# duckietown/gym-duckietown

Measured on NVIDIA H100. Metric: env-steps/sec (obs+reward+done) at N envs, 1/2/4/8 H100 vs CPU ref, higher is better.
Workload: dtype f64 logic / f32 raster / u8 obs

## Files before the change

### gym-duckietown_b200/csrc/dts_render.cu

```cuda
#include <algorithm>
#include <cstddef>
#include <cstdlib>
#include <type_traits>
#include <vector>

#include "dts_camera.cuh"
#include "dts_kernels.h"

namespace dts {

struct FishTab {
  const int32_t* src_xy;
  const short4* cbox;
  const short4* fbox;
  const int32_t* cell_start;
  const uint16_t* cell_bins;
  const int32_t* home_start;
  const int4* home_ent;
  int ext_x, ext_y;
};

struct PilTab {
  int W, H, ow, oh;
  int tx, ty;
  int band, cap;
  int pitch, ow3p;
  size_t smem;
  int32_t* tab;
};

namespace {

#ifndef DTS_STATS
#define DTS_STATS 0
#endif
#if DTS_STATS
#define DTS_COUNT(slot, n) do { if (lane == 0) atomicAdd(err + (slot), (n)); } while (0)
#else
#define DTS_COUNT(slot, n) do { } while (0)
#endif
constexpr int kThreads = 256;
constexpr int kRasterMinCtas = 3;
constexpr int kSoloMinCtas = 3;
constexpr int kFlatMinCtas = 4;
constexpr int kGeoWarps = 1;
constexpr int kGeoMinCtas = 32;
constexpr int kWarps = kThreads / 32;
constexpr int kBinW = 8, kBinH = 4;
constexpr int kCFX = 4, kCFY = 2;
constexpr int kCoarseW = kBinW * kCFX, kCoarseH = kBinH * kCFY;
constexpr int kStage = 32;
constexpr float kGuard = 4.0f;
constexpr int kSub = 64;
constexpr int kTessTris = 98;
__host__ __device__ constexpr int tile_draw_ids(bool tess) { return tess ? kTessTris : 2; }
__host__ __device__ constexpr int agent_item(int n_tiles, int n_objects) { return 1 + n_tiles + n_objects; }
__host__ __device__ constexpr int sample_x(int s) { return s == 0 ? 24 : (s == 1 ? 56 : (s == 2 ? 8 : 40)); }
__host__ __device__ constexpr int sample_y(int s) { return s == 0 ? 8 : (s == 1 ? 24 : (s == 2 ? 40 : 56)); }

struct Vtx { float cx, cy, cz, cw, r, g, b, u, v; };

struct __align__(16) PrimRec {
  int32_t X0, Y0, X1, Y1;
  int32_t X2, Y2, X3, Y3;
  float z0, zx, zy;
  int32_t id;
  float q0, qx, qy, u0;
  float ux, uy, v0, vx;
  float vy;
  int32_t ltq;
  uint32_t tex;
  float r0;
  float rx, ry, g0, gx;
  float gy, b0, bx, by;
};
static_assert(sizeof(PrimRec) == 128, "PrimRec must be 128 bytes");
static_assert(offsetof(PrimRec, q0) == 48 && offsetof(PrimRec, vy) == 80 && offsetof(PrimRec, rx) == 96, "PrimRec word groups");

struct __align__(16) BinRec {
  int32_t E0[4], A[4], B[4];
  float z0, zx, zy;
  int32_t id;
  int32_t x0, y0;
  uint32_t prim_flags;
  int32_t kind;
};
static_assert(sizeof(BinRec) == 80, "BinRec layout");
constexpr int kKindQuad = 1;
constexpr int kKindGround = 2;
constexpr int kKindTiny = 4;
constexpr int kKindFlat = 8;
constexpr unsigned kNoPrim = 0xffffu;

struct Xform { float MV[12], N[9]; };

struct __align__(16) FrameCtx {
  double V[12];
  float P00, P11, P22, P23;
  int32_t n_prims, n_lat, overflow, pad;
};

struct __align__(16) GeoWarp {
  int32_t unlit, pad_[3];
  RenderEp ep;
  double V[12];
  float P00, P11, P22, P23;
  Xform x;
  Vtx corners[4];
  Vtx poly[2][12];
};
using Shared = GeoWarp;

__device__ __forceinline__ void model_view(const double* V, double tx, double ty, double tz, double sc, double c,
                                           double s, Xform& x, int lane) {
  __syncwarp();
  if (lane < 12) {
    const int r = lane >> 2, k = lane & 3;
    if (k < 3) {
      const double R0 = k == 0 ? c : (k == 1 ? 0.0 : s), R1 = k == 1 ? 1.0 : 0.0, R2 = k == 0 ? -s : (k == 1 ? 0.0 : c);
      const double a = V[4 * r + 0] * R0 + V[4 * r + 1] * R1 + V[4 * r + 2] * R2;
      x.MV[4 * r + k] = (float)(a * sc);
      x.N[3 * r + k] = (float)(sc == 1.0 ? a : a / sc);
    } else {
      x.MV[4 * r + 3] = (float)(V[4 * r + 0] * tx + V[4 * r + 1] * ty + V[4 * r + 2] * tz + V[4 * r + 3]);
    }
  }
  __syncwarp();
}


__device__ __forceinline__ Vtx shade_vertex(const Xform& x, const Shared& sh, float px, float py, float pz, float nx,
                                            float ny, float nz, float cr, float cg, float cb, float u, float v) {
  float e[3], ne[3];
#pragma unroll
  for (int r = 0; r < 3; r++) {
    float t = x.MV[4 * r] * px;
    t = t + x.MV[4 * r + 1] * py;
    t = t + x.MV[4 * r + 2] * pz;
    e[r] = t + x.MV[4 * r + 3];
    float q = x.N[3 * r] * nx;
    q = q + x.N[3 * r + 1] * ny;
    ne[r] = q + x.N[3 * r + 2] * nz;
  }
  const float* lp = sh.ep.light_eye;
  float lx, ly, lz;
  if (lp[3] == 0.0f) { lx = lp[0]; ly = lp[1]; lz = lp[2]; }
  else { lx = lp[0] - e[0]; ly = lp[1] - e[1]; lz = lp[2] - e[2]; }
  float len = lx * lx;
  len = len + ly * ly;
  len = len + lz * lz;
  len = sqrtf(len);
  float ndl = 0.0f;
  if (len > 0.0f) {
    lx = lx / len; ly = ly / len; lz = lz / len;
    ndl = ne[0] * lx;
    ndl = ndl + ne[1] * ly;
    ndl = ndl + ne[2] * lz;
    if (!(ndl > 0.0f)) ndl = 0.0f;
  }
  Vtx o;
  const float col[3] = {cr, cg, cb};
  float lit[3];
#pragma unroll
  for (int k = 0; k < 3; k++) {
    float s = 0.3f + sh.ep.ambient[k];
    s = s + ndl * sh.ep.diffuse[k];
    const float c = sh.unlit ? col[k] : col[k] * s;
    lit[k] = c < 0.0f ? 0.0f : (c > 1.0f ? 1.0f : c);
  }
  o.r = lit[0]; o.g = lit[1]; o.b = lit[2];
  o.u = u; o.v = v;
  o.cx = sh.P00 * e[0];
  o.cy = sh.P11 * e[1];
  o.cz = sh.P22 * e[2] + sh.P23;
  o.cw = -e[2];
  return o;
}

__device__ __forceinline__ float plane_dist(const Vtx& a, int pl) {
  switch (pl) {
    case 0: return a.cz + a.cw;
    case 1: return a.cw - a.cz;
    case 2: return a.cx + kGuard * a.cw;
    case 3: return kGuard * a.cw - a.cx;
    case 4: return a.cy + kGuard * a.cw;
    default: return kGuard * a.cw - a.cy;
  }
}

__device__ __forceinline__ int classify(const Vtx& a, const Vtx& b, const Vtx& c) {
  const Vtx* v[3] = {&a, &b, &c};
  int out[6] = {0, 0, 0, 0, 0, 0}, need = 0;
#pragma unroll
  for (int k = 0; k < 3; k++) {
    const float x = v[k]->cx, y = v[k]->cy, z = v[k]->cz, w = v[k]->cw;
    out[0] += !(z + w >= 0.0f); out[1] += !(w - z >= 0.0f);
    out[2] += x < -w; out[3] += x > w; out[4] += y < -w; out[5] += y > w;
    need |= !(x + kGuard * w >= 0.0f) | !(kGuard * w - x >= 0.0f) | !(y + kGuard * w >= 0.0f) |
            !(kGuard * w - y >= 0.0f);
  }
  need |= out[0] | out[1];
#pragma unroll
  for (int p = 0; p < 6; p++) if (out[p] == 3) return 2;
  return need ? 1 : 0;
}

struct EmitCtx {
  const DTexture* textures;
  GeoWarp* gw;
  FrameCtx* ctx;
  PrimRec* prims;
  int max_prims, W, H;
};

__device__ __noinline__ bool setup_and_emit(const EmitCtx& ec, const Vtx& a, const Vtx& b, const Vtx& c, int id,
                                            int tex, int lat, const Vtx* d = nullptr) {
  const Vtx* vs[3] = {&a, &b, &c};
  int X[3], Y[3];
  float zw[3], q[3];
  const float Wf = (float)ec.W, Hf = (float)ec.H;
#pragma unroll
  for (int k = 0; k < 3; k++) {
    const float iw = 1.0f / vs[k]->cw;
    const float nx = vs[k]->cx * iw, ny = vs[k]->cy * iw, nz = vs[k]->cz * iw;
    const float sx = (nx * 0.5f + 0.5f) * Wf;
    const float sy = (0.5f - ny * 0.5f) * Hf;
    X[k] = (int)rintf(sx * 64.0f);
    Y[k] = (int)rintf(sy * 64.0f);
    zw[k] = nz * 0.5f + 0.5f;
    q[k] = iw;
  }
// ... 25 lines not shown
    const int ex[3] = {x1 - x0, x2 - x1, x0 - x2}, ey[3] = {y1 - y0, y2 - y1, y0 - y2};
    const int ax[3] = {0, x1 - x0, x2 - x0}, ay[3] = {0, y1 - y0, y2 - y0};
    int e00[3];
#pragma unroll
    for (int k = 0; k < 3; k++) {
      const int bias = (ey[k] > 0 || (ey[k] == 0 && ex[k] < 0)) ? 0 : 1;
      e00[k] = ex[k] * (py0 * kSub - y0 - ay[k]) - ey[k] * (px0 * kSub - x0 - ax[k]) - bias;
    }
    bool any = false;
    for (int py = 0; py <= py1 - py0; py++)
      for (int px = 0; px <= px1 - px0; px++) {
#pragma unroll
        for (int s = 0; s < 4; s++) {
          const int sx = px * kSub + sample_x(s), sy = py * kSub + sample_y(s);
          const int e0 = e00[0] + ex[0] * sy - ey[0] * sx, e1 = e00[1] + ex[1] * sy - ey[1] * sx, e2 = e00[2] + ex[2] * sy - ey[2] * sx;
          any |= (e0 | e1 | e2) >= 0;
        }
      }
    if (!any) return true;
  }
  PrimRec r;
  r.X0 = x0; r.Y0 = y0; r.X1 = x1; r.Y1 = y1; r.X2 = x2; r.Y2 = y2; r.X3 = x0; r.Y3 = y0;
  const float dx1 = (float)(x1 - x0) * 0.015625f, dy1 = (float)(y1 - y0) * 0.015625f;
  const float dx2 = (float)(x2 - x0) * 0.015625f, dy2 = (float)(y2 - y0) * 0.015625f;
  const float areaf = dx1 * dy2 - dx2 * dy1;
  const float ia = 1.0f / areaf;
  const Vtx* p0 = vs[0]; const Vtx* p1 = vs[i1]; const Vtx* p2 = vs[i2];
  const float q0 = q[0], q1 = q[i1], q2 = q[i2];
  const float v0[7] = {zw[0], q0, p0->u * q0, p0->v * q0, p0->r * q0, p0->g * q0, p0->b * q0};
  const float v1[7] = {zw[i1], q1, p1->u * q1, p1->v * q1, p1->r * q1, p1->g * q1, p1->b * q1};
  const float v2[7] = {zw[i2], q2, p2->u * q2, p2->v * q2, p2->r * q2, p2->g * q2, p2->b * q2};
  float f0[7], fx[7], fy[7];
#pragma unroll
  for (int at = 0; at < 7; at++) {
    const float d1 = v1[at] - v0[at], d2 = v2[at] - v0[at];
    f0[at] = v0[at];
    fx[at] = (d1 * dy2 - d2 * dy1) * ia;
    fy[at] = (d2 * dx1 - d1 * dx2) * ia;
  }
  r.z0 = f0[0]; r.zx = fx[0]; r.zy = fy[0];
  r.q0 = f0[1]; r.qx = fx[1]; r.qy = fy[1];
  r.u0 = f0[2]; r.ux = fx[2]; r.uy = fy[2];
  r.v0 = f0[3]; r.vx = fx[3]; r.vy = fy[3];
  r.r0 = f0[4]; r.rx = fx[4]; r.ry = fy[4];
  r.g0 = f0[5]; r.gx = fx[5]; r.gy = fy[5];
  r.b0 = f0[6]; r.bx = fx[6]; r.by = fy[6];
  r.id = id;
  r.ltq = (lat + 1) | ((tex + 1) << 16);
  r.tex = tex >= 0 ? ec.textures[tex].info : 0u;
  if (d) {
    r.ltq |= 1 << 24;
    r.X1 = qx[1]; r.Y1 = qy[1]; r.X2 = qx[2]; r.Y2 = qy[2]; r.X3 = qx[3]; r.Y3 = qy[3];
  }
  const int slot = atomicAdd(&ec.ctx->n_prims, 1);
  if (slot >= ec.max_prims) { ec.ctx->overflow = 1; return true; }
  const int4* src = reinterpret_cast<const int4*>(&r);
  int4* dst = reinterpret_cast<int4*>(ec.prims + slot);
#pragma unroll
  for (int k = 0; k < 8; k++) dst[k] = src[k];
  return true;
}

__device__ __forceinline__ Vtx clip_lerp(const Vtx& in, const Vtx& out, float din, float dout) {
  const float t = din / (din - dout);
  Vtx o;
  const float* a = reinterpret_cast<const float*>(&in);
  const float* b = reinterpret_cast<const float*>(&out);
  float* c = reinterpret_cast<float*>(&o);
#pragma unroll
  for (int k = 0; k < 9; k++) { const float d = b[k] - a[k]; c[k] = a[k] + t * d; }
  return o;
}

__device__ __forceinline__ void clip_and_emit_warp(const EmitCtx& ec, const Vtx& a, const Vtx& b, const Vtx& c, int id,
                                                   int tex, int lat, int lane) {
  for (int p2 = 0; p2 < 6; p2++) {
    const int cnt = !(plane_dist(a, p2) >= 0.0f) + !(plane_dist(b, p2) >= 0.0f) + !(plane_dist(c, p2) >= 0.0f);
    if (cnt == 3) return;
  }
  GeoWarp& g = *ec.gw;
  __syncwarp();
  if (lane == 0) { g.poly[0][0] = a; g.poly[0][1] = b; g.poly[0][2] = c; }
  __syncwarp();
  int n = 3, cur = 0;
  for (int pl = 0; pl < 6; pl++) {
    const Vtx* P = g.poly[cur];
    const float dk = lane < n ? plane_dist(P[lane], pl) : 0.0f;
    const bool in1 = dk >= 0.0f;
    const unsigned valid = (1u << n) - 1u;
    const unsigned out_mask = __ballot_sync(0xffffffffu, lane < n && !in1);
    if (!out_mask) continue;
    const int k2 = (lane + 1 == n) ? 0 : lane + 1;
    const float dn = __shfl_sync(0xffffffffu, dk, k2 & 31);
    const bool in2 = dn >= 0.0f;
    const bool cross = lane < n && (in1 != in2);
    const unsigned keep_mask = __ballot_sync(0xffffffffu, lane < n && in1) & valid;
    const unsigned cross_mask = __ballot_sync(0xffffffffu, cross) & valid;
    const unsigned below = (1u << lane) - 1u;
    int pos = __popc(keep_mask & below) + __popc(cross_mask & below);
    Vtx* T = g.poly[cur ^ 1];
    if (lane < n) {
      if (in1) T[pos++] = P[lane];
      if (in1 && !in2) T[pos] = clip_lerp(P[lane], P[k2], dk, dn);
      else if (!in1 && in2) T[pos] = clip_lerp(P[k2], P[lane], dn, dk);
    }
    n = __popc(keep_mask) + __popc(cross_mask);
    cur ^= 1;
// ... 446 lines not shown
  out |= (P11 * cy_ + cz_) * hy > rad * 1.01f;
  out |= (-P11 * cy_ + cz_) * hy > rad * 1.01f;
  return out;
}
__device__ __forceinline__ void eye_point(const double* V, double wx, double wy, double wz, float& ex, float& ey, float& ez) {
  ex = (float)(V[0] * wx + V[1] * wy + V[2] * wz + V[3]);
  ey = (float)(V[4] * wx + V[5] * wy + V[6] * wz + V[7]);
  ez = (float)(V[8] * wx + V[9] * wy + V[10] * wz + V[11]);
}

struct ItemPose { int dyn_kind; float opx, opz, orot; bool agent_item; };
__device__ __forceinline__ bool item_visible(const DState& S, const DMap& m, const RenderCfg& rc, const FrameCtx& ctx, int env,
                                             int item, ItemPose& ip) {
  const int n_tiles = m.grid_w * m.grid_h;
  ip.dyn_kind = 0; ip.opx = 0.f; ip.opz = 0.f; ip.orot = 0.f;
  ip.agent_item = item == agent_item(n_tiles, m.n_objects);
  if (item > agent_item(n_tiles, m.n_objects)) return false;
  if (ip.agent_item && (!(rc.mode & DTS_RENDER_TOP_DOWN) || m.agent.tri_count == 0)) return false;
  if (item >= 1 && item <= n_tiles) {
    const int t = item - 1, ti = t / m.grid_h, tj = t - ti * m.grid_h;
    if (m.tile_kind[tj * m.grid_w + ti] < 0) return false;
    const double ts = m.tile_size;
    float ex, ey, ez;
    eye_point(ctx.V, (ti + 0.5) * ts, 0.0, (tj + 0.5) * ts, ex, ey, ez);
    if (sphere_outside(ctx.P00, ctx.P11, ex, ey, ez, (float)(ts * 0.7071067811865476) * 1.001f + 1e-4f)) return false;
  } else if (item > n_tiles) {
    const int o = item - 1 - n_tiles;
    if (!ip.agent_item && (S.rep[env].hidden[o >> 5] >> (o & 31) & 1u)) return false;
    const DObject& ob = ip.agent_item ? m.agent : m.objects[o];
    ip.opx = ob.pos[0]; ip.opz = ob.pos[2]; ip.orot = ob.y_rot_deg;
    if (ip.agent_item) {
      ip.opx = (float)S.pos_x[env]; ip.opz = (float)S.pos_z[env];
      ip.orot = (float)(S.angle[env] * 180.0 / 3.141592653589793);
    }
    if (ob.dyn_slot >= 0) {
      ip.dyn_kind = m.dyn[ob.dyn_slot].kind;
      if (ip.dyn_kind != DTS_DYN_TRAFFICLIGHT) {
        const size_t nd = m.n_dyn, ne = rc.n_envs;
        ip.opx = (float)m.dyn_state[((size_t)DTS_DYN_PX * nd + ob.dyn_slot) * ne + env];
        ip.opz = (float)m.dyn_state[((size_t)DTS_DYN_PZ * nd + ob.dyn_slot) * ne + env];
        ip.orot = (float)m.dyn_state[((size_t)DTS_DYN_YROT * nd + ob.dyn_slot) * ne + env];
      }
    }
    double sn, cs;
    sincos((double)ip.orot * kDeg2Rad, &sn, &cs);
    const double sc = (double)ob.scale, ccx = ob.centre[0], ccy = ob.centre[1], ccz = ob.centre[2];
    float ex, ey, ez;
    eye_point(ctx.V, (double)ip.opx + sc * (cs * ccx + sn * ccz), (double)ob.pos[1] + sc * ccy, (double)ip.opz + sc * (-sn * ccx + cs * ccz), ex, ey, ez);
    if (sphere_outside(ctx.P00, ctx.P11, ex, ey, ez, ob.bound_rad * ob.scale * 1.002f + 2e-4f)) return false;
  }
  return true;
}

__global__ void __launch_bounds__(256) k_cull(const DState S, const DMap* __restrict__ maps, RenderCfg rc, FrameMem fm, int items_max) {
  const size_t g = blockIdx.x * (size_t)blockDim.x + threadIdx.x;
  const int item = (int)(g / rc.n_envs), slot = (int)(g - (size_t)item * rc.n_envs);
  bool vis = false;
  int env = 0;
  if (item < items_max && slot < n_listed(rc.env_list, rc.env_count, rc.n_envs)) {
    env = listed_env(rc.env_list, slot);
    ItemPose ip;
    vis = item_visible(S, maps[S.map_id[env]], rc, fm.ctx[env], env, item, ip);
  }
  const unsigned m = __ballot_sync(0xffffffffu, vis);
  if (!m) return;
  const int lane = threadIdx.x & 31;
  int base = 0;
  if (lane == __ffs(m) - 1) base = atomicAdd(fm.work + kWorkGeoList, __popc(m));
  base = __shfl_sync(0xffffffffu, base, __ffs(m) - 1);
  if (vis) fm.geo_list[base + __popc(m & ((1u << lane) - 1u))] = make_uint2((unsigned)env, (unsigned)item);
}

template <bool kTess>
__device__ __forceinline__ void geometry_item(const DState& S, const DMap* __restrict__ maps, const RenderCfg& rc, const FrameMem& fm,
                                              int max_prims, int max_lat, int32_t* __restrict__ err, int env, int item, int lane,
                                              GeoWarp& sh) {
  const DMap& m = maps[S.map_id[env]];
  const int n_tiles = m.grid_w * m.grid_h;
  const bool seg = (rc.mode & DTS_RENDER_SEGMENT) != 0;
  const int W = rc.width, H = rc.height;
  FrameCtx& ctx = fm.ctx[env];
  ItemPose ip;
  if (!item_visible(S, m, rc, ctx, env, item, ip)) return;
  const bool agent_item = ip.agent_item;
  const int dyn_kind = ip.dyn_kind;
  const float opx = ip.opx, opz = ip.opz, orot = ip.orot;
  __syncwarp();
  for (int k = lane; k < (int)(sizeof(RenderEp) / 4); k += 32)
    reinterpret_cast<uint32_t*>(&sh.ep)[k] = reinterpret_cast<const uint32_t*>(&S.rep[env])[k];
  if (lane < 12) sh.V[lane] = ctx.V[lane];
  if (lane == 12) { sh.P00 = ctx.P00; sh.P11 = ctx.P11; sh.P22 = ctx.P22; sh.P23 = ctx.P23; sh.unlit = seg ? 1 : 0; }
  __syncwarp();
  EmitCtx ec{m.textures, &sh, &ctx, fm.prims + (size_t)env * max_prims, max_prims, W, H};
  float4* lat_tab = fm.lat + (size_t)env * max_lat * 64;
  const int tris_per_tile = tile_draw_ids(kTess);
  Xform& x = sh.x;
  if (item == 0) {
    model_view(sh.V, 0.0, 0.0, 0.0, 1.0, 1.0, 0.0, x, lane);
    const float gy = (float)(-0.8 * 0.01);
    const float P[4][3] = {{-50.f, gy, 50.f}, {-50.f, gy, -50.f}, {50.f, gy, -50.f}, {50.f, gy, 50.f}};
    const float magenta[3] = {255.f, 0.f, 255.f};
    const float* g = seg ? magenta : sh.ep.ground;
    const int pl_ = lane & 3;
    const Vtx mine = shade_vertex(x, sh, P[pl_][0], P[pl_][1], P[pl_][2], 0.f, 1.f, 0.f, g[0], g[1], g[2], 0.f, 0.f);
    if (lane < 4) sh.corners[lane] = mine;
    __syncwarp();
    process_triangle_uniform(ec, sh.corners[0], sh.corners[1], sh.corners[2], 0, -1, -1, lane);
    process_triangle_uniform(ec, sh.corners[0], sh.corners[2], sh.corners[3], 1, -1, -1, lane);
  } else if (item <= n_tiles) {
    const int t = item - 1, ti = t / m.grid_h, tj = t - ti * m.grid_h;
    const int idx = tj * m.grid_w + ti;
    const int quarter = (m.tile_angle[idx] + 2) & 3;
    const double cs = quarter == 0 ? 1.0 : (quarter == 2 ? -1.0 : 0.0), sn = quarter == 1 ? 1.0 : (quarter == 3 ? -1.0 : 0.0);
    const double ts = m.tile_size;
    model_view(sh.V, (double)(float)((ti + 0.5) * ts), 0.0, (double)(float)((tj + 0.5) * ts), 1.0, cs, sn, x, lane);
    int tex = m.tile_tex[idx];
    if (seg && tex >= 0) tex = m.tex_segment[tex];
    const int base_id = 2 + tris_per_tile * t;
    if (!kTess) {
      const int ca = (lane == 1 || lane == 2) ? 7 : 0, cb = (lane >= 2) ? 7 : 0;
      const float lx = (float)(-ts / 2 + ((double)ca / 7.0) * ts), lz = (float)(-ts / 2 + ((double)cb / 7.0) * ts);
      const Vtx v = shade_vertex(x, sh, lx, 0.0f, lz, 0.f, 1.f, 0.f, 1.f, 1.f, 1.f, (float)((double)ca / 7.0),
                                 (float)(1.0 - (double)cb / 7.0));
      const unsigned four = 0xFu;
      bool culled4 = false;
      culled4 |= (__ballot_sync(0xffffffffu, !(v.cz + v.cw >= 0.0f)) & four) == four;
      culled4 |= (__ballot_sync(0xffffffffu, !(v.cw - v.cz >= 0.0f)) & four) == four;
      culled4 |= (__ballot_sync(0xffffffffu, v.cx < -v.cw) & four) == four;
      culled4 |= (__ballot_sync(0xffffffffu, v.cx > v.cw) & four) == four;
      culled4 |= (__ballot_sync(0xffffffffu, v.cy < -v.cw) & four) == four;
      culled4 |= (__ballot_sync(0xffffffffu, v.cy > v.cw) & four) == four;
      if (culled4) return;
    }
    Vtx lv[2];
    int outside[6] = {0, 0, 0, 0, 0, 0};
#pragma unroll
    for (int h = 0; h < 2; h++) {
      const int vi = lane + 32 * h, a = vi >> 3, b = vi & 7;
      const float lx = (float)(-ts / 2 + ((double)a / 7.0) * ts), lz = (float)(-ts / 2 + ((double)b / 7.0) * ts);
      lv[h] = shade_vertex(x, sh, lx, 0.0f, lz, 0.f, 1.f, 0.f, 1.f, 1.f, 1.f, (float)((double)a / 7.0),
                           (float)(1.0 - (double)b / 7.0));
      const Vtx& v = lv[h];
      outside[0] += !(v.cz + v.cw >= 0.0f); outside[1] += !(v.cw - v.cz >= 0.0f);
      outside[2] += v.cx < -v.cw; outside[3] += v.cx > v.cw; outside[4] += v.cy < -v.cw; outside[5] += v.cy > v.cw;
    }
    if (kTess) {
      bool culled = false;
#pragma unroll
      for (int p = 0; p < 6; p++) culled |= __all_sync(0xffffffffu, outside[p] == 2);
      if (culled) return;
    }
    if (!kTess) {
      int slot = 0;
      if (lane == 0) slot = atomicAdd(&ctx.n_lat, 1);
      slot = __shfl_sync(0xffffffffu, slot, 0);
      if (slot >= max_lat) { if (lane == 0) ctx.overflow = 1; return; }
#pragma unroll
      for (int h = 0; h < 2; h++) {
        const int vi = lane + 32 * h;
        lat_tab[slot * 64 + vi] = make_float4(lv[h].r, lv[h].g, lv[h].b, 0.0f);
        int corner = -1;
        if (vi == 0) corner = 0; else if (vi == 56) corner = 1; else if (vi == 63) corner = 2; else if (vi == 7) corner = 3;
        if (corner >= 0) { Vtx c = lv[h]; c.r = 0.f; c.g = 0.f; c.b = 0.f; sh.corners[corner] = c; }
      }
      __syncwarp();
      bool as_quad = false;
      if (classify(sh.corners[0], sh.corners[1], sh.corners[2]) == 0 && classify(sh.corners[0], sh.corners[2], sh.corners[3]) == 0) {
        if (lane == 0) as_quad = setup_and_emit(ec, sh.corners[0], sh.corners[1], sh.corners[2], base_id, tex, slot, &sh.corners[3]);
        as_quad = __shfl_sync(0xffffffffu, (int)as_quad, 0) != 0;
      }
      if (!as_quad) {
        process_triangle_uniform(ec, sh.corners[0], sh.corners[1], sh.corners[2], base_id, tex, slot, lane);
        process_triangle_uniform(ec, sh.corners[0], sh.corners[2], sh.corners[3], base_id + 1, tex, slot, lane);
      }
      } else {
      for (int k0 = 0; k0 < kTessTris; k0 += 32) {
        const int k = k0 + lane;
        Vtx v[3];
        if (k < kTessTris) {
          const int quad = k >> 1, half = k & 1, a = quad / 7, b = quad - 7 * a;
#pragma unroll
          for (int j = 0; j < 3; j++) {
            const int aa = j == 0 ? a : (j == 1 ? a + 1 : (half == 0 ? a + 1 : a));
            const int bb = j == 0 ? b : (j == 1 ? (half == 0 ? b : b + 1) : b + 1);
            const float lx = (float)(-ts / 2 + ((double)aa / 7.0) * ts), lz = (float)(-ts / 2 + ((double)bb / 7.0) * ts);
            v[j] = shade_vertex(x, sh, lx, 0.0f, lz, 0.f, 1.f, 0.f, 1.f, 1.f, 1.f, (float)((double)aa / 7.0),
                                (float)(1.0 - (double)bb / 7.0));
          }
        }
        process_triangle_lanes(ec, k < kTessTris, v[0], v[1], v[2], base_id + k, tex, -1, lane);
          }
    }
  } else {
    const int o = item - 1 - n_tiles;
    const DObject& ob = agent_item ? m.agent : m.objects[o];
    int alt_from = -2;
    if (dyn_kind == DTS_DYN_TRAFFICLIGHT) {
      const size_t nd = m.n_dyn, ne = rc.n_envs;
      if (m.dyn_state[((size_t)DTS_DYN_SHOWN * nd + m.dyn[ob.dyn_slot].tl_first) * ne + env] != 0.0) alt_from = ob.alt_from;
    }
    double sn, cs;
    sincos((double)orot * kDeg2Rad, &sn, &cs);
    model_view(sh.V, (double)opx, (double)ob.pos[1], (double)opz, (double)ob.scale, cs, sn, x, lane);
    int base_id = 2 + tris_per_tile * n_tiles;
    for (int q = 0; q < o; q++) base_id += m.objects[q].tri_count;
    for (int k0 = 0; k0 < ob.tri_count; k0 += 32) {
      const int k = k0 + lane;
      Vtx v[3];
      int ttex = -1;
      if (k < ob.tri_count) {
        const size_t ti = (size_t)ob.tri_offset + k;
        const float* p = m.tri_pos + ti * 9;
        const float* n = m.tri_nrm + ti * 9;
        const float* uv = m.tri_uv + ti * 6;
        const float* c = m.tri_col + ti * 9;
#pragma unroll
        for (int j = 0; j < 3; j++)
          v[j] = shade_vertex(x, sh, p[3 * j], p[3 * j + 1], p[3 * j + 2], n[3 * j], n[3 * j + 1], n[3 * j + 2],
                              c[3 * j], c[3 * j + 1], c[3 * j + 2], uv[2 * j], uv[2 * j + 1]);
        ttex = m.tri_tex[ti];
        if (ttex == alt_from) ttex = ob.alt_to;
        if (seg) ttex = ob.seg_tex;
      }
      process_triangle_lanes(ec, k < ob.tri_count, v[0], v[1], v[2], base_id + k, ttex, -1, lane);
      }
  }
  if (lane == 0 && ctx.overflow) { atomicOr(err, 1); *reinterpret_cast<volatile int32_t*>(fm.status) = 1; }
}

template <bool kTess>
__global__ void __launch_bounds__(kGeoWarps * 32, kGeoMinCtas)
k_geometry(const DState S, const DMap* __restrict__ maps, RenderCfg rc, FrameMem fm, int max_prims, int max_lat,
           int32_t* __restrict__ err) {
  __shared__ GeoWarp gws[kGeoWarps];
  const int lane = threadIdx.x & 31, wib = threadIdx.x >> 5;
  const int n_list = fm.work[kWorkGeoList];
  for (int wi = blockIdx.x * kGeoWarps + wib; wi < n_list; wi += gridDim.x * kGeoWarps) {
    const uint2 e = fm.geo_list[wi];
    geometry_item<kTess>(S, maps, rc, fm, max_prims, max_lat, err, (int)e.x, (int)e.y, lane, gws[wib]);
  }
}

constexpr int kBinWarps = 4;
constexpr int kCountMask = 0xfffff, kGroundInc = 1 << 20;
constexpr int kFlatBin = -0x7fffffff - 1;
template <bool kFish, bool kListed>
__global__ void __launch_bounds__(kBinWarps * 32)
k_bin(RenderCfg rc, FrameMem fm, FishTab ft, int max_prims, int max_pairs, int32_t* __restrict__ err) {
  extern __shared__ int bin_smem[];
  __shared__ int s_total, s_base, s_ok;
  const int lane = threadIdx.x & 31, wib = threadIdx.x >> 5, tid = threadIdx.x;
  if (kListed && (int)blockIdx.x >= __ldg(rc.env_count)) return;
  const int env = kListed ? __ldg(rc.env_list + blockIdx.x) : (int)blockIdx.x, nthr = blockDim.x;
  const int W = rc.width, H = rc.height;
  const int cbins_x = (W + kCoarseW - 1) / kCoarseW, cbins_y = (H + kCoarseH - 1) / kCoarseH, cbins = cbins_x * cbins_y;
  int* cnt = bin_smem;
  int* start = cnt + cbins;
  const PrimRec* prims = fm.prims + (size_t)env * max_prims;
  uint32_t* pairs = fm.pairs;
  const int n = min(fm.ctx[env].n_prims, max_prims);
  for (int pass = 0; pass < 2; pass++) {
    for (int b = tid; b < cbins; b += nthr) cnt[b] = 0;
    __syncthreads();
    for (int p0 = wib * 32; p0 < n; p0 += nthr) {
      const int p = p0 + lane;
      const bool have = p < n;
      int qx[4] = {0, 0, 0, 0}, qy[4] = {0, 0, 0, 0}, nv = 3, ginc = 1;
      if (have) {
        const int4 w0 = __ldg(reinterpret_cast<const int4*>(prims + p));
        const int4 w1 = __ldg(reinterpret_cast<const int4*>(prims + p) + 1);
        qx[0] = w0.x; qx[1] = w0.z; qx[2] = w1.x; qx[3] = w1.z;
        qy[0] = w0.y; qy[1] = w0.w; qy[2] = w1.y; qy[3] = w1.w;
        nv = ((__ldg(&prims[p].ltq) >> 24) & 1) ? 4 : 3;
        if (__ldg(&prims[p].id) < 2) ginc = 1 + kGroundInc;
      }
      const int minx = min(min(qx[0], qx[1]), min(qx[2], qx[3])), maxx = max(max(qx[0], qx[1]), max(qx[2], qx[3]));
      const int miny = min(min(qy[0], qy[1]), min(qy[2], qy[3])), maxy = max(max(qy[0], qy[1]), max(qy[2], qy[3]));
      const int pminx = max(minx >> 6, 0), pmaxx = min(maxx >> 6, W - 1), pminy = max(miny >> 6, 0), pmaxy = min(maxy >> 6, H - 1);
      const int bx0 = pminx / kCoarseW, by0 = pminy / kCoarseH, bx1 = pmaxx / kCoarseW, by1 = pmaxy / kCoarseH;
      const bool big = have && (bx1 - bx0 + 1) * (by1 - by0 + 1) > 8;
      if (have && !big) {
        if (kFish) {
          for (int cy = by0; cy <= by1; cy++)
            for (int cx = bx0; cx <= bx1; cx++) {
              const int c = cy * cbins_x + cx;
              for (int q = ft.cell_start[c]; q < ft.cell_start[c + 1]; q++) {
                const int b = ft.cell_bins[q];
                const short4 cb = ft.cbox[b];
                if (pmaxx < cb.x || pminx > cb.z || pmaxy < cb.y || pminy > cb.w) continue;
                if (cx != max(bx0, cb.x / kCoarseW) || cy != max(by0, cb.y / kCoarseH)) continue;
                const int pos = atomicAdd(&cnt[b], ginc) & kCountMask;
                if (pass == 1) pairs[start[b] + pos] = (uint32_t)p | ((uint32_t)b << 16);
              }
// ... 1297 lines not shown
  slot = t;
  return "";
}

std::string debug_frame_copy(const Renderer& r, int env, double* V, float* P, int32_t* counts, float* lattice_by_cell,
                             int n_cells) {
  if (!r.frame) return "nothing rendered yet";
  if (r.flags & DTS_FLAG_TESSELLATE) return "dts_debug_frame reads the analytic-tile lattice (tile mode 1)";
  const FrameMem& fm = r.fm;
  const int max_prims = r.max_prims, max_lat = r.max_lat, tris_per_tile = tile_draw_ids(false);
  FrameCtx c;
  if (cudaMemcpy(&c, fm.ctx + env, sizeof c, cudaMemcpyDeviceToHost) != cudaSuccess) return "debug_frame_copy failed";
  for (int k = 0; k < 12; k++) V[k] = c.V[k];
  P[0] = c.P00; P[1] = c.P11; P[2] = c.P22; P[3] = c.P23;
  counts[0] = c.n_prims; counts[1] = c.n_lat; counts[2] = c.overflow; counts[3] = 0;
  cudaMemcpy(&counts[3], fm.work + kWorkPairPool, sizeof(int32_t), cudaMemcpyDeviceToHost);
  const int np = c.n_prims < max_prims ? c.n_prims : max_prims;
  std::vector<PrimRec> prims(np > 0 ? np : 1);
  std::vector<float4> lat((size_t)max_lat * 64);
  int rc = 0;
  if (np && cudaMemcpy(prims.data(), fm.prims + (size_t)env * max_prims, (size_t)np * sizeof(PrimRec), cudaMemcpyDeviceToHost) != cudaSuccess) rc = 1;
  if (cudaMemcpy(lat.data(), fm.lat + (size_t)env * max_lat * 64, (size_t)max_lat * 64 * sizeof(float4), cudaMemcpyDeviceToHost) != cudaSuccess) rc = 1;
  for (int k = 0; k < n_cells * 64 * 3; k++) lattice_by_cell[k] = nanf("");
  for (int p = 0; p < np && !rc; p++) {
    const int slot = (prims[p].ltq & 0xffff) - 1;
    if (slot < 0 || slot >= max_lat) continue;
    const int cell = (prims[p].id - 2) / tris_per_tile;
    if (cell < 0 || cell >= n_cells) continue;
    for (int v = 0; v < 64; v++) {
      lattice_by_cell[(cell * 64 + v) * 3 + 0] = lat[slot * 64 + v].x;
      lattice_by_cell[(cell * 64 + v) * 3 + 1] = lat[slot * 64 + v].y;
      lattice_by_cell[(cell * 64 + v) * 3 + 2] = lat[slot * 64 + v].z;
    }
  }
  return rc ? "debug_frame_copy failed" : "";
}

int launch_render(const Renderer& r, const DState& S, const DMap* maps, const RenderCfg& rc, void* obs_any, const GatherTab& gather,
                  int32_t* err_flag, int32_t* status_dev, cudaEvent_t* marks, int mark_level, cudaStream_t st) {
  uint8_t* obs = reinterpret_cast<uint8_t*>(obs_any);
  const FishTab* lut = (rc.mode & DTS_RENDER_RECTIFY) ? &r.rect
                     : ((rc.flags & DTS_FLAG_DISTORTION) && !(rc.mode & DTS_RENDER_PINHOLE)) ? &r.fish : nullptr;
  const bool fisheye = lut != nullptr;
  const FishTab ft = fisheye ? *lut : FishTab{};
  FrameMem fm = r.fm;
  fm.status = status_dev;
  int mk = 0;
  auto mark = [&]() { if (marks && (mark_level >= 2 || mk == 3 || mk == 4)) cudaEventRecord(marks[mk], st); mk++; };
  cudaMemsetAsync(fm.work, 0, 256, st);
  mark();
  k_frame_setup<<<(rc.n_envs + 127) / 128, 128, 0, st>>>(S, maps, rc, fm);
  mark();
  const size_t pairs_total = (size_t)rc.n_envs * r.items_max;
  k_cull<<<(unsigned)((pairs_total + 255) / 256), 256, 0, st>>>(S, maps, rc, fm, r.items_max);
  const auto geometry = rc.tessellate ? k_geometry<true> : k_geometry<false>;
  geometry<<<r.sms * kGeoMinCtas / kGeoWarps, kGeoWarps * 32, 0, st>>>(S, maps, rc, fm, r.max_prims, r.max_lat, err_flag);
  mark();
  const size_t bin_smem_bytes = (size_t)2 * r.cbins * sizeof(int);
  const int bin_grid = rc.n_envs;
  const int bin_threads = r.cbins > 128 ? kBinWarps * 32 : 32;
  const auto bin = rc.env_list ? (fisheye ? k_bin<true, true> : k_bin<false, true>) : (fisheye ? k_bin<true, false> : k_bin<false, false>);
  if (bin_smem_bytes > 48 * 1024)
    cudaFuncSetAttribute(bin, cudaFuncAttributeMaxDynamicSharedMemorySize, (int)bin_smem_bytes);
  bin<<<bin_grid, bin_threads, bin_smem_bytes, st>>>(rc, fm, ft, r.max_prims, r.pool, err_flag);
  mark();
  const bool wrap = (rc.obs_layout | rc.obs_dtype) != 0;
  int launches = 5;
  if (lean_output(rc.obs_layout, rc.obs_dtype, rc.width)) {
    const auto solo = fisheye ? k_raster_solo<true> : k_raster_solo<false>;
    const auto flat = fisheye ? k_raster_flat<true> : k_raster_flat<false>;
    solo<<<r.sms * kSoloMinCtas, kThreads, 0, st>>>(S, maps, rc, fm, ft, obs, r.max_prims, r.max_lat);
    flat<<<r.sms * kFlatMinCtas, kThreads, 0, st>>>(S, maps, rc, fm, ft, obs, r.max_prims, r.max_lat, err_flag);
    launches += 2;
  }
  static bool smem_opt_in = false;
  if (!smem_opt_in) {
    cudaFuncSetAttribute(k_raster<true, true>, cudaFuncAttributeMaxDynamicSharedMemorySize, (int)kRasterSmem);
    cudaFuncSetAttribute(k_raster<false, true>, cudaFuncAttributeMaxDynamicSharedMemorySize, (int)kRasterSmem);
    cudaFuncSetAttribute(k_raster<true, false>, cudaFuncAttributeMaxDynamicSharedMemorySize, (int)kRasterSmem);
    cudaFuncSetAttribute(k_raster<false, false>, cudaFuncAttributeMaxDynamicSharedMemorySize, (int)kRasterSmem);
    smem_opt_in = true;
  }
  const auto raster = fisheye ? (wrap ? k_raster<true, true> : k_raster<false, true>) : (wrap ? k_raster<true, false> : k_raster<false, false>);
  raster<<<r.sms * kRasterMinCtas, kThreads, kRasterSmem, st>>>(S, maps, rc, fm, ft, gather, obs, r.max_prims, r.pool, r.max_lat, err_flag);
  mark();
  mark();
  return launches;
}

}
```

Before: 2.554 million.

## Add per-env tile kernel processing one tile per lane for non-tessellated maps

Adds a k_tiles kernel for the non-tessellated path. One warp handles one env and each lane takes one tile. Lanes cull tiles by bounding sphere and corner frustum tests, compute the model-view transform themselves, and emit quads, clipping triangles only when needed. The ground plane is drawn in this kernel too. k_cull now skips tile items and the ground when not tessellating, so the per-item warp geometry kernel handles only objects. Primitive slot allocation is aggregated per warp with one atomic. The aim is to remove a warp-per-tile pass in which most lanes sit idle, at the cost of an extra launch, more shared memory per block, and a serial per-tile loop for lighting writes.

New measurement: 2.669 million (median of 6 runs). 4.5% higher.

```diff
diff --git a/gym-duckietown_b200/csrc/dts_render.cu b/gym-duckietown_b200/csrc/dts_render.cu
--- a/gym-duckietown_b200/csrc/dts_render.cu
+++ b/gym-duckietown_b200/csrc/dts_render.cu
@@ -45,6 +45,8 @@
 constexpr int kFlatMinCtas = 4;
 constexpr int kGeoWarps = 1;
 constexpr int kGeoMinCtas = 32;
+constexpr int kTileWarps = 4;
+constexpr int kTileMinCtas = 4;
 constexpr int kWarps = kThreads / 32;
 constexpr int kBinW = 8, kBinH = 4;
 constexpr int kCFX = 4, kCFY = 2;
@@ -111,20 +113,21 @@
 };
 using Shared = GeoWarp;
 
+__device__ __forceinline__ void model_view_entry(const double* V, double tx, double ty, double tz, double sc, double c,
+                                                 double s, int r, int k, Xform& x) {
+  if (k < 3) {
+    const double R0 = k == 0 ? c : (k == 1 ? 0.0 : s), R1 = k == 1 ? 1.0 : 0.0, R2 = k == 0 ? -s : (k == 1 ? 0.0 : c);
+    const double a = V[4 * r + 0] * R0 + V[4 * r + 1] * R1 + V[4 * r + 2] * R2;
+    x.MV[4 * r + k] = (float)(a * sc);
+    x.N[3 * r + k] = (float)(sc == 1.0 ? a : a / sc);
+  } else {
+    x.MV[4 * r + 3] = (float)(V[4 * r + 0] * tx + V[4 * r + 1] * ty + V[4 * r + 2] * tz + V[4 * r + 3]);
+  }
+}
 __device__ __forceinline__ void model_view(const double* V, double tx, double ty, double tz, double sc, double c,
                                            double s, Xform& x, int lane) {
   __syncwarp();
-  if (lane < 12) {
-    const int r = lane >> 2, k = lane & 3;
-    if (k < 3) {
-      const double R0 = k == 0 ? c : (k == 1 ? 0.0 : s), R1 = k == 1 ? 1.0 : 0.0, R2 = k == 0 ? -s : (k == 1 ? 0.0 : c);
-      const double a = V[4 * r + 0] * R0 + V[4 * r + 1] * R1 + V[4 * r + 2] * R2;
-      x.MV[4 * r + k] = (float)(a * sc);
-      x.N[3 * r + k] = (float)(sc == 1.0 ? a : a / sc);
-    } else {
-      x.MV[4 * r + 3] = (float)(V[4 * r + 0] * tx + V[4 * r + 1] * ty + V[4 * r + 2] * tz + V[4 * r + 3]);
-    }
-  }
+  if (lane < 12) model_view_entry(V, tx, ty, tz, sc, c, s, lane >> 2, lane & 3, x);
   __syncwarp();
 }
 
@@ -177,6 +180,18 @@
   return o;
 }
 
+__device__ __forceinline__ Vtx tile_vertex(const Xform& x, const Shared& sh, double ts, int a, int b) {
+  const float lx = (float)(-ts / 2 + ((double)a / 7.0) * ts), lz = (float)(-ts / 2 + ((double)b / 7.0) * ts);
+  return shade_vertex(x, sh, lx, 0.0f, lz, 0.f, 1.f, 0.f, 1.f, 1.f, 1.f, (float)((double)a / 7.0), (float)(1.0 - (double)b / 7.0));
+}
+struct TilePose { double tx, tz, cs, sn; };
+__device__ __forceinline__ TilePose tile_pose(const DMap& m, int ti, int tj) {
+  const int quarter = (m.tile_angle[tj * m.grid_w + ti] + 2) & 3;
+  const double ts = m.tile_size;
+  return TilePose{(double)(float)((ti + 0.5) * ts), (double)(float)((tj + 0.5) * ts),
+                  quarter == 0 ? 1.0 : (quarter == 2 ? -1.0 : 0.0), quarter == 1 ? 1.0 : (quarter == 3 ? -1.0 : 0.0)};
+}
+
 __device__ __forceinline__ float plane_dist(const Vtx& a, int pl) {
   switch (pl) {
     case 0: return a.cz + a.cw;
@@ -308,7 +323,11 @@
     r.ltq |= 1 << 24;
     r.X1 = qx[1]; r.Y1 = qy[1]; r.X2 = qx[2]; r.Y2 = qy[2]; r.X3 = qx[3]; r.Y3 = qy[3];
   }
-  const int slot = atomicAdd(&ec.ctx->n_prims, 1);
+  const unsigned act = __activemask();
+  const int lane = threadIdx.x & 31, leader = __ffs(act) - 1;
+  int slot = 0;
+  if (lane == leader) slot = atomicAdd(&ec.ctx->n_prims, __popc(act));
+  slot = __shfl_sync(act, slot, leader) + __popc(act & ((1u << lane) - 1u));
   if (slot >= ec.max_prims) { ec.ctx->overflow = 1; return true; }
   const int4* src = reinterpret_cast<const int4*>(&r);
   int4* dst = reinterpret_cast<int4*>(ec.prims + slot);
@@ -861,29 +880,53 @@
   return true;
 }
 
-__global__ void __launch_bounds__(256) k_cull(const DState S, const DMap* __restrict__ maps, RenderCfg rc, FrameMem fm, int items_max) {
+__global__ void __launch_bounds__(256) k_cull(const DState S, const DMap* __restrict__ maps, RenderCfg rc, FrameMem fm, int items_max,
+                                              int32_t* __restrict__ err) {
   const size_t g = blockIdx.x * (size_t)blockDim.x + threadIdx.x;
   const int item = (int)(g / rc.n_envs), slot = (int)(g - (size_t)item * rc.n_envs);
   bool vis = false;
   int env = 0;
   if (item < items_max && slot < n_listed(rc.env_list, rc.env_count, rc.n_envs)) {
     env = listed_env(rc.env_list, slot);
+    const DMap& m = maps[S.map_id[env]];
     ItemPose ip;
-    vis = item_visible(S, maps[S.map_id[env]], rc, fm.ctx[env], env, item, ip);
+    vis = (rc.tessellate || item > m.grid_w * m.grid_h) && item_visible(S, m, rc, fm.ctx[env], env, item, ip);
   }
   const unsigned m = __ballot_sync(0xffffffffu, vis);
   if (!m) return;
   const int lane = threadIdx.x & 31;
+  DTS_COUNT(28, __popc(m));
   int base = 0;
   if (lane == __ffs(m) - 1) base = atomicAdd(fm.work + kWorkGeoList, __popc(m));
   base = __shfl_sync(0xffffffffu, base, __ffs(m) - 1);
   if (vis) fm.geo_list[base + __popc(m & ((1u << lane) - 1u))] = make_uint2((unsigned)env, (unsigned)item);
 }
 
+__device__ __forceinline__ void load_geo_warp(GeoWarp& sh, const DState& S, const FrameCtx& ctx, int env, bool seg, int lane) {
+  for (int k = lane; k < (int)(sizeof(RenderEp) / 4); k += 32)
+    reinterpret_cast<uint32_t*>(&sh.ep)[k] = reinterpret_cast<const uint32_t*>(&S.rep[env])[k];
+  if (lane < 12) sh.V[lane] = ctx.V[lane];
+  if (lane == 12) { sh.P00 = ctx.P00; sh.P11 = ctx.P11; sh.P22 = ctx.P22; sh.P23 = ctx.P23; sh.unlit = seg ? 1 : 0; }
+  __syncwarp();
+}
+
+__device__ __forceinline__ void draw_ground(const EmitCtx& ec, GeoWarp& sh, bool seg, int lane) {
+  model_view(sh.V, 0.0, 0.0, 0.0, 1.0, 1.0, 0.0, sh.x, lane);
+  const float gy = (float)(-0.8 * 0.01);
+  const float P[4][3] = {{-50.f, gy, 50.f}, {-50.f, gy, -50.f}, {50.f, gy, -50.f}, {50.f, gy, 50.f}};
+  const float magenta[3] = {255.f, 0.f, 255.f};
+  const float* g = seg ? magenta : sh.ep.ground;
+  const int pl_ = lane & 3;
+  const Vtx mine = shade_vertex(sh.x, sh, P[pl_][0], P[pl_][1], P[pl_][2], 0.f, 1.f, 0.f, g[0], g[1], g[2], 0.f, 0.f);
+  if (lane < 4) sh.corners[lane] = mine;
+  __syncwarp();
+  process_triangle_uniform(ec, sh.corners[0], sh.corners[1], sh.corners[2], 0, -1, -1, lane);
+  process_triangle_uniform(ec, sh.corners[0], sh.corners[2], sh.corners[3], 1, -1, -1, lane);
+}
+
 template <bool kTess>
 __device__ __forceinline__ void geometry_item(const DState& S, const DMap* __restrict__ maps, const RenderCfg& rc, const FrameMem& fm,
-                                              int max_prims, int max_lat, int32_t* __restrict__ err, int env, int item, int lane,
-                                              GeoWarp& sh) {
+                                              int max_prims, int32_t* __restrict__ err, int env, int item, int lane, GeoWarp& sh) {
   const DMap& m = maps[S.map_id[env]];
   const int n_tiles = m.grid_w * m.grid_h;
   const bool seg = (rc.mode & DTS_RENDER_SEGMENT) != 0;
@@ -895,110 +938,50 @@
   const int dyn_kind = ip.dyn_kind;
   const float opx = ip.opx, opz = ip.opz, orot = ip.orot;
   __syncwarp();
-  for (int k = lane; k < (int)(sizeof(RenderEp) / 4); k += 32)
-    reinterpret_cast<uint32_t*>(&sh.ep)[k] = reinterpret_cast<const uint32_t*>(&S.rep[env])[k];
-  if (lane < 12) sh.V[lane] = ctx.V[lane];
-  if (lane == 12) { sh.P00 = ctx.P00; sh.P11 = ctx.P11; sh.P22 = ctx.P22; sh.P23 = ctx.P23; sh.unlit = seg ? 1 : 0; }
-  __syncwarp();
+  load_geo_warp(sh, S, ctx, env, seg, lane);
   EmitCtx ec{m.textures, &sh, &ctx, fm.prims + (size_t)env * max_prims, max_prims, W, H};
-  float4* lat_tab = fm.lat + (size_t)env * max_lat * 64;
   const int tris_per_tile = tile_draw_ids(kTess);
   Xform& x = sh.x;
-  if (item == 0) {
-    model_view(sh.V, 0.0, 0.0, 0.0, 1.0, 1.0, 0.0, x, lane);
-    const float gy = (float)(-0.8 * 0.01);
-    const float P[4][3] = {{-50.f, gy, 50.f}, {-50.f, gy, -50.f}, {50.f, gy, -50.f}, {50.f, gy, 50.f}};
-    const float magenta[3] = {255.f, 0.f, 255.f};
-    const float* g = seg ? magenta : sh.ep.ground;
-    const int pl_ = lane & 3;
-    const Vtx mine = shade_vertex(x, sh, P[pl_][0], P[pl_][1], P[pl_][2], 0.f, 1.f, 0.f, g[0], g[1], g[2], 0.f, 0.f);
-    if (lane < 4) sh.corners[lane] = mine;
-    __syncwarp();
-    process_triangle_uniform(ec, sh.corners[0], sh.corners[1], sh.corners[2], 0, -1, -1, lane);
-    process_triangle_uniform(ec, sh.corners[0], sh.corners[2], sh.corners[3], 1, -1, -1, lane);
-  } else if (item <= n_tiles) {
-    const int t = item - 1, ti = t / m.grid_h, tj = t - ti * m.grid_h;
-    const int idx = tj * m.grid_w + ti;
-    const int quarter = (m.tile_angle[idx] + 2) & 3;
-    const double cs = quarter == 0 ? 1.0 : (quarter == 2 ? -1.0 : 0.0), sn = quarter == 1 ? 1.0 : (quarter == 3 ? -1.0 : 0.0);
-    const double ts = m.tile_size;
-    model_view(sh.V, (double)(float)((ti + 0.5) * ts), 0.0, (double)(float)((tj + 0.5) * ts), 1.0, cs, sn, x, lane);
-    int tex = m.tile_tex[idx];
-    if (seg && tex >= 0) tex = m.tex_segment[tex];
-    const int base_id = 2 + tris_per_tile * t;
-    if (!kTess) {
-      const int ca = (lane == 1 || lane == 2) ? 7 : 0, cb = (lane >= 2) ? 7 : 0;
-      const float lx = (float)(-ts / 2 + ((double)ca / 7.0) * ts), lz = (float)(-ts / 2 + ((double)cb / 7.0) * ts);
-      const Vtx v = shade_vertex(x, sh, lx, 0.0f, lz, 0.f, 1.f, 0.f, 1.f, 1.f, 1.f, (float)((double)ca / 7.0),
-                                 (float)(1.0 - (double)cb / 7.0));
-      const unsigned four = 0xFu;
-      bool culled4 = false;
-      culled4 |= (__ballot_sync(0xffffffffu, !(v.cz + v.cw >= 0.0f)) & four) == four;
-      culled4 |= (__ballot_sync(0xffffffffu, !(v.cw - v.cz >= 0.0f)) & four) == four;
-      culled4 |= (__ballot_sync(0xffffffffu, v.cx < -v.cw) & four) == four;
-      culled4 |= (__ballot_sync(0xffffffffu, v.cx > v.cw) & four) == four;
-      culled4 |= (__ballot_sync(0xffffffffu, v.cy < -v.cw) & four) == four;
-      culled4 |= (__ballot_sync(0xffffffffu, v.cy > v.cw) & four) == four;
-      if (culled4) return;
-    }
-    Vtx lv[2];
-    int outside[6] = {0, 0, 0, 0, 0, 0};
-#pragma unroll
-    for (int h = 0; h < 2; h++) {
-      const int vi = lane + 32 * h, a = vi >> 3, b = vi & 7;
-      const float lx = (float)(-ts / 2 + ((double)a / 7.0) * ts), lz = (float)(-ts / 2 + ((double)b / 7.0) * ts);
-      lv[h] = shade_vertex(x, sh, lx, 0.0f, lz, 0.f, 1.f, 0.f, 1.f, 1.f, 1.f, (float)((double)a / 7.0),
-                           (float)(1.0 - (double)b / 7.0));
-      const Vtx& v = lv[h];
-      outside[0] += !(v.cz + v.cw >= 0.0f); outside[1] += !(v.cw - v.cz >= 0.0f);
-      outside[2] += v.cx < -v.cw; outside[3] += v.cx > v.cw; outside[4] += v.cy < -v.cw; outside[5] += v.cy > v.cw;
-    }
-    if (kTess) {
-      bool culled = false;
-#pragma unroll
-      for (int p = 0; p < 6; p++) culled |= __all_sync(0xffffffffu, outside[p] == 2);
-      if (culled) return;
-    }
-    if (!kTess) {
-      int slot = 0;
-      if (lane == 0) slot = atomicAdd(&ctx.n_lat, 1);
-      slot = __shfl_sync(0xffffffffu, slot, 0);
-      if (slot >= max_lat) { if (lane == 0) ctx.overflow = 1; return; }
-#pragma unroll
-      for (int h = 0; h < 2; h++) {
-        const int vi = lane + 32 * h;
-        lat_tab[slot * 64 + vi] = make_float4(lv[h].r, lv[h].g, lv[h].b, 0.0f);
-        int corner = -1;
-        if (vi == 0) corner = 0; else if (vi == 56) corner = 1; else if (vi == 63) corner = 2; else if (vi == 7) corner = 3;
-        if (corner >= 0) { Vtx c = lv[h]; c.r = 0.f; c.g = 0.f; c.b = 0.f; sh.corners[corner] = c; }
-      }
-      __syncwarp();
-      bool as_quad = false;
-      if (classify(sh.corners[0], sh.corners[1], sh.corners[2]) == 0 && classify(sh.corners[0], sh.corners[2], sh.corners[3]) == 0) {
-        if (lane == 0) as_quad = setup_and_emit(ec, sh.corners[0], sh.corners[1], sh.corners[2], base_id, tex, slot, &sh.corners[3]);
-        as_quad = __shfl_sync(0xffffffffu, (int)as_quad, 0) != 0;
-      }
-      if (!as_quad) {
-        process_triangle_uniform(ec, sh.corners[0], sh.corners[1], sh.corners[2], base_id, tex, slot, lane);
-        process_triangle_uniform(ec, sh.corners[0], sh.corners[2], sh.corners[3], base_id + 1, tex, slot, lane);
-      }
+  if (item <= n_tiles) {
+    if constexpr (kTess) {
+      if (item == 0) {
+        draw_ground(ec, sh, seg, lane);
       } else {
-      for (int k0 = 0; k0 < kTessTris; k0 += 32) {
-        const int k = k0 + lane;
-        Vtx v[3];
-        if (k < kTessTris) {
-          const int quad = k >> 1, half = k & 1, a = quad / 7, b = quad - 7 * a;
-#pragma unroll
-          for (int j = 0; j < 3; j++) {
-            const int aa = j == 0 ? a : (j == 1 ? a + 1 : (half == 0 ? a + 1 : a));
-            const int bb = j == 0 ? b : (j == 1 ? (half == 0 ? b : b + 1) : b + 1);
-            const float lx = (float)(-ts / 2 + ((double)aa / 7.0) * ts), lz = (float)(-ts / 2 + ((double)bb / 7.0) * ts);
-            v[j] = shade_vertex(x, sh, lx, 0.0f, lz, 0.f, 1.f, 0.f, 1.f, 1.f, 1.f, (float)((double)aa / 7.0),
-                                (float)(1.0 - (double)bb / 7.0));
+        const int t = item - 1, ti = t / m.grid_h, tj = t - ti * m.grid_h;
+        const int idx = tj * m.grid_w + ti;
+        const TilePose tp = tile_pose(m, ti, tj);
+        const double ts = m.tile_size;
+        model_view(sh.V, tp.tx, 0.0, tp.tz, 1.0, tp.cs, tp.sn, x, lane);
+        int tex = m.tile_tex[idx];
+        if (seg && tex >= 0) tex = m.tex_segment[tex];
+        const int base_id = 2 + tris_per_tile * t;
+        int outside[6] = {0, 0, 0, 0, 0, 0};
+#pragma unroll
+        for (int h = 0; h < 2; h++) {
+          const int vi = lane + 32 * h;
+          const Vtx v = tile_vertex(x, sh, ts, vi >> 3, vi & 7);
+          outside[0] += !(v.cz + v.cw >= 0.0f); outside[1] += !(v.cw - v.cz >= 0.0f);
+          outside[2] += v.cx < -v.cw; outside[3] += v.cx > v.cw; outside[4] += v.cy < -v.cw; outside[5] += v.cy > v.cw;
+        }
+        bool culled = false;
+#pragma unroll
+        for (int p = 0; p < 6; p++) culled |= __all_sync(0xffffffffu, outside[p] == 2);
+        if (culled) return;
+        for (int k0 = 0; k0 < kTessTris; k0 += 32) {
+          const int k = k0 + lane;
+          Vtx v[3];
+          if (k < kTessTris) {
+            const int quad = k >> 1, half = k & 1, a = quad / 7, b = quad - 7 * a;
+#pragma unroll
+            for (int j = 0; j < 3; j++) {
+              const int aa = j == 0 ? a : (j == 1 ? a + 1 : (half == 0 ? a + 1 : a));
+              const int bb = j == 0 ? b : (j == 1 ? (half == 0 ? b : b + 1) : b + 1);
+              v[j] = tile_vertex(x, sh, ts, aa, bb);
+            }
           }
+          process_triangle_lanes(ec, k < kTessTris, v[0], v[1], v[2], base_id + k, tex, -1, lane);
         }
-        process_triangle_lanes(ec, k < kTessTris, v[0], v[1], v[2], base_id + k, tex, -1, lane);
-          }
+      }
     }
   } else {
     const int o = item - 1 - n_tiles;
@@ -1039,15 +1022,105 @@
 
 template <bool kTess>
 __global__ void __launch_bounds__(kGeoWarps * 32, kGeoMinCtas)
-k_geometry(const DState S, const DMap* __restrict__ maps, RenderCfg rc, FrameMem fm, int max_prims, int max_lat,
-           int32_t* __restrict__ err) {
+k_geometry(const DState S, const DMap* __restrict__ maps, RenderCfg rc, FrameMem fm, int max_prims, int32_t* __restrict__ err) {
   __shared__ GeoWarp gws[kGeoWarps];
   const int lane = threadIdx.x & 31, wib = threadIdx.x >> 5;
   const int n_list = fm.work[kWorkGeoList];
   for (int wi = blockIdx.x * kGeoWarps + wib; wi < n_list; wi += gridDim.x * kGeoWarps) {
     const uint2 e = fm.geo_list[wi];
-    geometry_item<kTess>(S, maps, rc, fm, max_prims, max_lat, err, (int)e.x, (int)e.y, lane, gws[wib]);
-  }
+    geometry_item<kTess>(S, maps, rc, fm, max_prims, err, (int)e.x, (int)e.y, lane, gws[wib]);
+  }
+}
+
+struct TileLanes {
+  Xform x[32];
+  Vtx c[32][4];
+};
+__global__ void __launch_bounds__(kTileWarps * 32, kTileMinCtas)
+k_tiles(const DState S, const DMap* __restrict__ maps, RenderCfg rc, FrameMem fm, int max_prims, int max_lat, int32_t* __restrict__ err) {
+  __shared__ GeoWarp gws[kTileWarps];
+  __shared__ TileLanes tls[kTileWarps];
+  const int lane = threadIdx.x & 31, wib = threadIdx.x >> 5;
+  const int slot = blockIdx.x * kTileWarps + wib;
+  if (slot >= n_listed(rc.env_list, rc.env_count, rc.n_envs)) return;
+  const int env = listed_env(rc.env_list, slot);
+  GeoWarp& sh = gws[wib];
+  TileLanes& tl = tls[wib];
+  const DMap& m = maps[S.map_id[env]];
+  FrameCtx& ctx = fm.ctx[env];
+  const bool seg = (rc.mode & DTS_RENDER_SEGMENT) != 0;
+  load_geo_warp(sh, S, ctx, env, seg, lane);
+  const EmitCtx ec{m.textures, &sh, &ctx, fm.prims + (size_t)env * max_prims, max_prims, rc.width, rc.height};
+  float4* lat_tab = fm.lat + (size_t)env * max_lat * 64;
+  const int n_tiles = m.grid_w * m.grid_h;
+  const double ts = m.tile_size;
+  for (int t0 = 0; t0 < n_tiles; t0 += 32) {
+    const int t = t0 + lane, ti = t / m.grid_h, tj = t - ti * m.grid_h, idx = tj * m.grid_w + ti;
+    bool live = false;
+    if (t < n_tiles && m.tile_kind[idx] >= 0) {
+      float ex, ey, ez;
+      eye_point(sh.V, (ti + 0.5) * ts, 0.0, (tj + 0.5) * ts, ex, ey, ez);
+      live = !sphere_outside(sh.P00, sh.P11, ex, ey, ez, (float)(ts * 0.7071067811865476) * 1.001f + 1e-4f);
+    }
+#if DTS_STATS
+    const unsigned in_sphere = __ballot_sync(0xffffffffu, live);
+    DTS_COUNT(29, __popc(in_sphere));
+#endif
+    Vtx* cn = tl.c[lane];
+    if (live) {
+      const TilePose tp = tile_pose(m, ti, tj);
+      Xform x;
+#pragma unroll
+      for (int e = 0; e < 12; e++) model_view_entry(sh.V, tp.tx, 0.0, tp.tz, 1.0, tp.cs, tp.sn, e >> 2, e & 3, x);
+      tl.x[lane] = x;
+      int out[6] = {0, 0, 0, 0, 0, 0};
+#pragma unroll
+      for (int k = 0; k < 4; k++) {
+        Vtx v = tile_vertex(x, sh, ts, (k == 1 || k == 2) ? 7 : 0, k >= 2 ? 7 : 0);
+        out[0] += !(v.cz + v.cw >= 0.0f); out[1] += !(v.cw - v.cz >= 0.0f);
+        out[2] += v.cx < -v.cw; out[3] += v.cx > v.cw; out[4] += v.cy < -v.cw; out[5] += v.cy > v.cw;
+        v.r = 0.f; v.g = 0.f; v.b = 0.f;
+        cn[k] = v;
+      }
+#pragma unroll
+      for (int p = 0; p < 6; p++) live &= out[p] != 4;
+    }
+    const unsigned lit = __ballot_sync(0xffffffffu, live);
+    if (!lit) continue;
+    int lat = 0;
+    if (lane == 0) lat = atomicAdd(&ctx.n_lat, __popc(lit));
+    lat = __shfl_sync(0xffffffffu, lat, 0) + __popc(lit & ((1u << lane) - 1u));
+    if (live && lat >= max_lat) { ctx.overflow = 1; live = false; }
+    int tex = -1;
+    bool clip = false;
+    if (live) {
+      tex = m.tile_tex[idx];
+      if (seg && tex >= 0) tex = m.tex_segment[tex];
+      clip = !(classify(cn[0], cn[1], cn[2]) == 0 && classify(cn[0], cn[2], cn[3]) == 0 &&
+               setup_and_emit(ec, cn[0], cn[1], cn[2], 2 + 2 * t, tex, lat, &cn[3]));
+    }
+    __syncwarp();
+    for (unsigned todo = __ballot_sync(0xffffffffu, live); todo; todo &= todo - 1) {
+      const int src = __ffs(todo) - 1, s = __shfl_sync(0xffffffffu, lat, src);
+#pragma unroll
+      for (int h = 0; h < 2; h++) {
+        const int vi = lane + 32 * h;
+        const Vtx v = tile_vertex(tl.x[src], sh, ts, vi >> 3, vi & 7);
+        lat_tab[s * 64 + vi] = make_float4(v.r, v.g, v.b, 0.0f);
+      }
+    }
+    for (unsigned todo = __ballot_sync(0xffffffffu, clip); todo; todo &= todo - 1) {
+      const int src = __ffs(todo) - 1, id = 2 + 2 * (t0 + src);
+      const int stex = __shfl_sync(0xffffffffu, tex, src), slat = __shfl_sync(0xffffffffu, lat, src);
+      const Vtx* c = tl.c[src];
+      process_triangle_uniform(ec, c[0], c[1], c[2], id, stex, slat, lane);
+      process_triangle_uniform(ec, c[0], c[2], c[3], id + 1, stex, slat, lane);
+    }
+    __syncwarp();
+  }
+  draw_ground(ec, sh, seg, lane);
+  __syncwarp();
+  if (lane == 0 && ctx.overflow) { atomicOr(err, 1); *reinterpret_cast<volatile int32_t*>(fm.status) = 1; }
 }
 
 constexpr int kBinWarps = 4;
@@ -2451,9 +2524,14 @@
   k_frame_setup<<<(rc.n_envs + 127) / 128, 128, 0, st>>>(S, maps, rc, fm);
   mark();
   const size_t pairs_total = (size_t)rc.n_envs * r.items_max;
-  k_cull<<<(unsigned)((pairs_total + 255) / 256), 256, 0, st>>>(S, maps, rc, fm, r.items_max);
+  k_cull<<<(unsigned)((pairs_total + 255) / 256), 256, 0, st>>>(S, maps, rc, fm, r.items_max, err_flag);
+  int launches = 5;
+  if (!rc.tessellate) {
+    k_tiles<<<(rc.n_envs + kTileWarps - 1) / kTileWarps, kTileWarps * 32, 0, st>>>(S, maps, rc, fm, r.max_prims, r.max_lat, err_flag);
+    launches++;
+  }
   const auto geometry = rc.tessellate ? k_geometry<true> : k_geometry<false>;
-  geometry<<<r.sms * kGeoMinCtas / kGeoWarps, kGeoWarps * 32, 0, st>>>(S, maps, rc, fm, r.max_prims, r.max_lat, err_flag);
+  geometry<<<r.sms * kGeoMinCtas / kGeoWarps, kGeoWarps * 32, 0, st>>>(S, maps, rc, fm, r.max_prims, err_flag);
   mark();
   const size_t bin_smem_bytes = (size_t)2 * r.cbins * sizeof(int);
   const int bin_grid = rc.n_envs;
@@ -2464,7 +2542,6 @@
   bin<<<bin_grid, bin_threads, bin_smem_bytes, st>>>(rc, fm, ft, r.max_prims, r.pool, err_flag);
   mark();
   const bool wrap = (rc.obs_layout | rc.obs_dtype) != 0;
-  int launches = 5;
   if (lean_output(rc.obs_layout, rc.obs_dtype, rc.width)) {
     const auto solo = fisheye ? k_raster_solo<true> : k_raster_solo<false>;
     const auto flat = fisheye ? k_raster_flat<true> : k_raster_flat<false>;
```
